# LouisBearing/BirdSoundClassif

Measured on AMD Instinct MI355X. Metric: clips/sec (3 s @ 22.05 kHz) detect fwd, higher is better.
Workload: dtype f32; 1 GPU; BASELINE.json configs[1]: 1xMI355X inference, batch=64 synthetic 3 s clips (PCM16 @22.05 kHz resident in HBM) through the HIP STFT front end + detector forward + device post-processing, detections returned to the host; batch_per_gpu=64, distinct_clips=64, lanes=2

## Files before the change

birdsoundclassif_amd/_lib.py:

```python
import ctypes as C
import os
import subprocess

_HERE = os.path.dirname(os.path.abspath(__file__))
LIB_PATH = os.environ.get('NBM_LIB') or os.path.join(_HERE, 'libnbm_hip.so')
CSRC = os.path.join(_HERE, 'csrc')

_lib = None


class GemmDesc(C.Structure):
    _fields_ = [('x', C.c_void_p), ('w', C.c_void_p), ('y', C.c_void_p),
                ('scale', C.c_void_p), ('shift', C.c_void_p), ('residual', C.c_void_p),
                ('x_gs', C.c_int64), ('w_gs', C.c_int64), ('y_gs', C.c_int64), ('res_gs', C.c_int64),
                ('groups', C.c_int),
                ('B', C.c_int), ('H', C.c_int), ('W', C.c_int), ('Cin', C.c_int),
                ('N', C.c_int),
                ('kh', C.c_int), ('kw', C.c_int), ('stride', C.c_int), ('pad', C.c_int),
                ('Ho', C.c_int), ('Wo', C.c_int),
                ('x_ld', C.c_int), ('w_ld', C.c_int), ('y_ld', C.c_int), ('res_ld', C.c_int),
                ('alpha', C.c_float), ('act', C.c_int), ('shift_per_row', C.c_int),
                ('up', C.c_void_p), ('up_H', C.c_int), ('up_W', C.c_int),
                ('rows', C.c_void_p), ('rows_blocks', C.c_void_p),
                ('rows_mode', C.c_int), ('rows_count', C.c_int), ('rows_TH', C.c_int), ('rows_TW', C.c_int),
# ... 76 lines not shown
    'nbm_upsample_bilinear_add': [_P, _I, _I, _I, _I, _P, _P, _I, _I, _P],
    'nbm_softmax_rows': [_P, _L, _I, _L, _P],
    'nbm_dwconv3x3': [_P, _I, _I, _I, _I, _I, _I, _P, _P, _P, _L, _P, _I, _I, _P],
    'nbm_silu': [_P, _P, _L, _P],
    'nbm_layernorm': [_P, _L, _I, _P, _P, _F, _P, _P],
    'nbm_mha_small': [_P, _P, _P, _I, _I, _I, _P, _I, _I, _I, _I, _I, _L, _L, _P, _F, _P],
    'nbm_mha_segments': [_P, _P, _P, _I, _I, _I, _P, _I, _I, _I, _I, _I, _I, _P, _P, _I, _F, _P],
    'nbm_pair_softmax': [_P, _L, _I, _I, _P, _I, _P],
    'nbm_rpn_decode': [_P, _P, _P, _I, _I, _I, _I, _I, _I, _P, _P, _P, _P],
    'nbm_nan_images': [_P, _I, _L, _P, _P],
    'nbm_rpn_select': [_P, _P, _P, _I, _I, _I, _I, _I, _P, _P, _P, _P, _P],
    'nbm_nms_batched': [_P, _P, _P, _I, _I, _F, _I, _P, _P, _P, _P, _P, _P, _P],
    'nbm_rpn_select_big_workspace': [_I, _I, C.POINTER(C.c_int64)],
    'nbm_rpn_select_big': [_P, _P, _P, _I, _I, _I, _I, _I, _P, _L, _P, _P, _P, _P, _P],
    'nbm_nms_big_workspace': [_I, _I, C.POINTER(C.c_int64)],
    'nbm_nms_big': [_P, _P, _P, _I, _I, _F, _I, _P, _L, _P, _P, _P, _P, _P],
    'nbm_roi_pool': [C.POINTER(RoiDesc), _P],
    'nbm_rcnn_post': [_P, _P, _I, _I, _P, _P, _I, _I, _I, _F, _F, _I, _P, _P, _P],
    'nbm_merge_collect': [_P, _P, _I, _I, _I, _I, _I, _L, _P, _P, _P, _P, _P, _P],
    'nbm_merge_nms_workspace': [_I, C.POINTER(C.c_int64)],
    'nbm_merge_nms': [_P, _P, _I, _F, _P, _L, _P, _P, _P],
    'nbm_merge_gather': [_P, _P, _P, _P, _P, _I, _P, _P, _P],
    'nbm_conv_dgrad': [C.POINTER(BwdDesc), _P],
    'nbm_conv_wgrad': [C.POINTER(BwdDesc), _P],
    'nbm_gemm_plan': [_I, _P, C.POINTER(GemmPlan)],
    'nbm_relu_bwd': [_P, _P, _P, _L, _P],
    'nbm_silu_bwd': [_P, _P, _P, _L, _P],
    'nbm_axpby': [_P, _P, _P, _F, _F, _L, _L, _P],
    'nbm_colsum': [_P, _L, _I, _I, _P, _P],
    'nbm_leaky_relu_bwd': [_P, _P, _P, _F, _L, _P],
    'nbm_layernorm_bwd': [_P, _P, _P, _L, _I, _F, _P, _P, _P, _P],
    'nbm_mha_small_bwd': [_P, _P, _P, _P, _I, _I, _I, _I, _P, _P, _P, _I, _I, _I, _P, _I, _I, _I, _I, _L, _L, _P, _F, _P],
    'nbm_zero_roi_windows': [_P, _I, _I, _I, _P, _P, _I, _I, _I, _P],
    'nbm_zero_pattern': [_P, _I, _I, _I, _I, _I, _P],
    'nbm_zero_tiles': [_P, _I, _I, _I, _I, _P, _I, _P, _P],
    'nbm_tiles_gather': [_P, _I, _I, _I, _I, _P, _I, _P, _P, _P],
    'nbm_tiles_scatter_add': [_P, _I, _I, _I, _I, _P, _I, _P, _P, _P],
    'nbm_proposal_iou': [_P, _P, _P, _I, _I, _I, _P, _P, _P],
    'nbm_anchor_targets': [_P, _I, _P, _P, _I, _I, _F, _F, _P, _P, _P, _P],
    'nbm_maxpool3x3s2_bwd': [_P, _P, _P, _I, _I, _I, _I, _I, _I, _P, _P, _P],
    'nbm_upsample_bilinear_bwd': [_P, _I, _I, _I, _I, _P, _I, _I, _I, _P],
    'nbm_tiles_upsample_bilinear_bwd_add': [_P, _I, _I, _I, _I, _P, _I, _P, _P, _I, _I, _P],
    'nbm_png_unfilter_gray8': [_P, _L, _I, _I, _I, _P, _L, _P, _P],
    'nbm_image_half_std_u8': [_P, _L, _I, _L, _P, _P],
    'nbm_randn_fill': [_U64, _L, _P, _P],
    'nbm_augment_batch': [_P, _P, _P, _I, _I, _I, _P, _P, _P, _P, _P, _P, _P],
    'nbm_u8_to_unit': [_P, _L, _P, _P],
    'nbm_wino_input': [_P, _I, _I, _I, _I, _P, _I, _P],
    'nbm_wino_output': [_P, _P, _P, _P, _I, _I, _I, _I, _I, _P, _I, _P, _P],
    'nbm_wino_outgrad': [_P, _I, _I, _I, _I, _P, _P, _I, _P],
    'nbm_wino_weight': [_P, _P, _I, _I, _I, _I, _P, _P],
    'nbm_wino_weight_grad': [_P, _P, _I, _I, _I, _P, _P],
    'nbm_wino23_rows': [_P, _I, _I, _I, _I, _P, _P],
    'nbm_wino23_conv_fused': [_P, _P, _P, _P, _P, _I, _I, _I, _I, _I, _I, _P, _I, _P],
    'nbm_wino23_rows_tiles': [_P, _I, _I, _I, _I, _P, _I, _P, _P, _P, _I, _P],
    'nbm_wino23_conv_fused_tiles': [_P, _P, _P, _P, _P, _I, _I, _I, _I, _I, _I, _P, _P, _I, _P, _P, _P],
    'nbm_roi_tiles': [_P, _P, _I, _I, _I, _I, _P, _P, _P, _I, _P, _P, _P],
    'nbm_wino23_input_tiles': [_P, _I, _I, _I, _I, _P, _I, _P, _P, _P],
    'nbm_wino23_outgrad_tiles': [_P, _I, _I, _I, _I, _P, _I, _P, _P, _P, _I, _P],
    'nbm_cell_outgrad': [_P, _I, _I, _I, _I, _I, _P, _P, _P],
    'nbm_cell_weight': [_P, _I, _I, _P, _I, _P, _I, _P],
    'nbm_cell_weight_fold': [_P, _P, _I, _I, _I, _I, _F, _P, _I, _P, _I, _P],
    'nbm_cell_weight_grad': [_P, _I, _I, _I, _P, _P],
    'nbm_cell_input': [_P, _I, _I, _I, _I, _I, _P, _I, _I, _P],
    'nbm_cell_input_up': [_P, _P, _I, _I, _I, _I, _I, _I, _I, _P, _I, _I, _P],
    'nbm_cell_patches': [_P, _I, _I, _I, _I, _I, _P, _I, _I, _P],
    'nbm_cell_patches_up': [_P, _P, _I, _I, _I, _I, _I, _I, _I, _P, _I, _I, _P],
    'nbm_cell_patches_up_cols': [_P, _P, _I, _I, _I, _I, _I, _I, _I, _P, _P],
    'nbm_cell_dgrad_output': [_P, _I, _I, _I, _I, _I, _P, _I, _I, _I, _P, _P],
    'nbm_cell_output': [_P, _P, _I, _I, _I, _I, _I, _P, _P],
    'nbm_weighted_sum': [_P, _P, _P, _P, _P, _L, _P],
    'nbm_weighted_sum_bwd': [_P, _P, _P, _P, _P, _P, _P, _P, _P, _L, _P],
    'nbm_softmax_rows_bwd': [_P, _P, _P, _L, _I, _F, _P],
    'nbm_pair_softmax_bwd': [_P, _P, _P, _L, _P],
    'nbm_dwconv3x3_bwd': [_P, _P, _P, _I, _I, _I, _I, _I, _I, _P, _P, _P, _I, _I, _P],
    'nbm_dwconv3x3_bwd_acc': [_P, _P, _I, _I, _I, _I, _I, _I, _P, _I, _I, _P],
    'nbm_film_fwd': [_P, _P, _P, _L, _I, _P],
    'nbm_film_bwd': [_P, _P, _P, _P, _P, _L, _I, _P],
    'nbm_bn_train_fwd': [_P, _L, _I, _P, _P, _F, _F, _P, _P, _P, _P, _P, _P, _P],
    'nbm_bn_train_bwd': [_P, _P, _L, _I, _P, _P, _P, _P, _P, _P, _P, _P],
    'nbm_roi_pool_bwd': [C.POINTER(C.c_void_p), C.POINTER(C.c_int), C.POINTER(C.c_int), _I, _I, _P, _P, _I, _I, _P, _P],
    'nbm_sqnorm_accum': [_P, _L, _P, _P],
    'nbm_adamw_step': [_P, _P, _P, _P, _L, _F, _F, _F, _F, _F, _I, _P, _F, _P],
}


def build(verbose=False):
    r = subprocess.run(['make', '-C', CSRC, '-j4'], capture_output=True, text=True)
    if verbose or r.returncode:
        print(r.stdout[-4000:], r.stderr[-4000:])
    if r.returncode:
        raise RuntimeError('building libnbm_hip.so failed')
    return LIB_PATH


def load():
    global _lib
    if _lib is not None:
        return _lib
    import torch
    if not os.path.isfile(LIB_PATH):
        raise RuntimeError(f'{LIB_PATH} is missing: build it with `python -c "import __graft_entry__ as g; g.build()"` '
                           '(the NBM hot path has no CPU / eager fallback)')
    lib = C.CDLL(LIB_PATH)
    lib.nbm_version.restype = C.c_char_p
    lib.nbm_version.argtypes = []
# ... 20 lines not shown
```

birdsoundclassif_amd/csrc/wino_fused.hip:

```cpp
#include "nbm_common.h"
#include "igemm_device.h"
#include <type_traits>

namespace {

constexpr int BK = 32;
constexpr int PITCH = 36;
constexpr int LIST_BM = 128;

struct WinoFusedParams {
  const float* R; const float* U; float* y;
  const float* scale; const float* shift; const float* mask;
  long long r_gs;
  int u_gs;
  int T, N, C, nk;
  int H, W, TH, TW, THW, WP;
  nbm_fastdiv fd_thw, fd_tw;
  int m_tiles, n_tiles, relu;
  const int* tiles; const int* n_blocks;
  const unsigned* blk_info;
};

__global__ __launch_bounds__(256) void wino23_rows_kernel(const float* __restrict__ x, int B, int H, int W, int C4,
                                                          int TH, int WP, float* __restrict__ R) {
  const long long per_plane = (long long)B * TH * WP * C4;
  const f32x4* x4 = reinterpret_cast<const f32x4*>(x);
  f32x4* r4 = reinterpret_cast<f32x4*>(R);
  const f32x4 zero = {0.f, 0.f, 0.f, 0.f};
  for (long long idx = blockIdx.x * 256ll + threadIdx.x; idx < per_plane; idx += (long long)gridDim.x * 256) {
    const int c = (int)(idx % C4);
    long long t = idx / C4;
    const int xp = (int)(t % WP);
    t /= WP;
    const int ty = (int)(t % TH), b = (int)(t / TH);
    const int ix = xp - 1;
    f32x4 d[4];
#pragma unroll
    for (int a = 0; a < 4; ++a) {
      const int iy = 2 * ty - 1 + a;
      const bool ok = (unsigned)iy < (unsigned)H && (unsigned)ix < (unsigned)W;
      d[a] = ok ? x4[(((long long)b * H + iy) * W + ix) * C4 + c] : zero;
    }
    r4[idx] = d[0] - d[2];
    r4[idx + per_plane] = d[1] + d[2];
    r4[idx + 2 * per_plane] = d[2] - d[1];
    r4[idx + 3 * per_plane] = d[1] - d[3];
  }
}

__global__ __launch_bounds__(256) void wino23_rows_tiles_kernel(const float* __restrict__ x, int B, int H, int W, int C4,
                                                                int TH, int TW, int WP, const int* __restrict__ tiles,
                                                                int n_entries, const int* __restrict__ n_blocks,
                                                                const unsigned* __restrict__ blk_info, float* __restrict__ R,
                                                                int pat_stride) {
  const int S = pat_stride, OHp = S > 0 ? (H + 2 - 3) / S + 1 : 0, OWp = S > 0 ? (W + 2 - 3) / S + 1 : 0;
  const long long per_plane = (long long)B * TH * WP * C4;
  const f32x4* x4 = reinterpret_cast<const f32x4*>(x);
  f32x4* r4 = reinterpret_cast<f32x4*>(R);
  const f32x4 zero = {0.f, 0.f, 0.f, 0.f};
  if (n_blocks) n_entries = min(n_entries, *n_blocks * LIST_BM);
  const long long total = (long long)n_entries * 4 * C4;
  for (long long idx = blockIdx.x * 256ll + threadIdx.x; idx < total; idx += (long long)gridDim.x * 256) {
    const int c = (int)(idx % C4);
    const long long t = idx / C4;
    const int k = (int)(t & 3), e = (int)(t >> 2);
    const int id = tiles[e];
    if (id < 0) continue;
    const unsigned pm = blk_info ? blk_info[e >> 7] & 0xffffu : 0xffffu;
    if ((k == 0 && !(pm & 0x1111u)) || (k == 3 && !(pm & 0x8888u))) continue;
    const int THW = TH * TW;
    const int b = id / THW, rem = id - b * THW;
    const int ty = rem / TW, tx = rem - ty * TW;
    const int xp = 2 * tx + k, ix = xp - 1;
    f32x4 d[4];
#pragma unroll
    for (int a = 0; a < 4; ++a) {
      const int iy = 2 * ty - 1 + a;
      bool ok = (unsigned)iy < (unsigned)H && (unsigned)ix < (unsigned)W &&
                !(a == 0 && !(pm & 0x000fu)) && !(a == 3 && !(pm & 0xf000u));
      if (S > 0 && ok && (iy + 1) % S < 3 && (iy + 1) / S < OHp && (ix + 1) % S < 3 && (ix + 1) / S < OWp) ok = false;
      d[a] = ok ? x4[(((long long)b * H + iy) * W + ix) * C4 + c] : zero;
    }
    const long long o = (((long long)b * TH + ty) * WP + xp) * C4 + c;
    if (pm & 0x000fu) r4[o] = d[0] - d[2];
    r4[o + per_plane] = d[1] + d[2];
    r4[o + 2 * per_plane] = d[2] - d[1];
    if (pm & 0xf000u) r4[o + 3 * per_plane] = d[1] - d[3];
  }
}

template <int BM, int BN, int WM, int WN>
__global__ __launch_bounds__(256, BN == 128 ? 1 : 2) void wino23_fused_kernel(const WinoFusedParams p) {
  constexpr int MT = WM / 32, NT = WN / 32;
  constexpr int WAVES_N = BN / WN;
  constexpr int AR = BM / 32, BR = BN / 32;
  static_assert((BM / WM) * WAVES_N == 4, "4 waves per workgroup");

  __shared__ __attribute__((aligned(16))) float lds[2 * (BM + BN) * PITCH];
  if constexpr (BN != 128) nbm_stagger_priority();
  float* As = lds;
  float* Bs = lds + 2 * BM * PITCH;

  const int wg = xcd_tile(gridDim.x, blockIdx.x);
  int tile_m = wg / p.n_tiles, tile_n = wg - tile_m * p.n_tiles;
  if (p.n_blocks) {
    const int j = blockIdx.x >> 3;
    tile_n = j % p.n_tiles;
    tile_m = (j / p.n_tiles) * 8 + (blockIdx.x & 7);
    if (tile_m >= p.m_tiles) return;
  }
  const int bm0 = tile_m * BM, bn0 = tile_n * BN;

  if (p.tiles) {
    if (p.n_blocks && tile_m >= *p.n_blocks) return;
    if (p.tiles[bm0] < 0) return;
  }
  auto tile_of = [&](int t) { return p.tiles ? p.tiles[t] : t; };
  const unsigned info = (p.tiles && p.blk_info) ? p.blk_info[tile_m] : 0x000fffffu;
  const unsigned plane_mask = info & 0xffffu, store_mask = (info >> 16) & 0xfu;

  const int tid = threadIdx.x, lane = tid & 63, wave = tid >> 6;
  const int wm0 = (wave / WAVES_N) * WM, wn0 = (wave % WAVES_N) * WN;
  const int lrow = lane & 31, lh = lane >> 5;
  const int c4 = tid & 7, r0 = tid >> 3;

  unsigned a_rel[AR], b_rel[BR];
  long long blk_base;
  {
    const int t = bm0 < p.T ? tile_of(bm0) : 0;
    const int bi = (int)nbm_fdiv((unsigned)t, p.fd_thw), rem = t - bi * p.THW;
    const int ty = (int)nbm_fdiv((unsigned)rem, p.fd_tw), tx = rem - ty * p.TW;
    blk_base = (((long long)bi * p.TH + ty) * p.WP + 2 * tx) * p.C;
  }
#pragma unroll
  for (int i = 0; i < AR; ++i) {
    const int t = bm0 + r0 + 32 * i < p.T ? tile_of(bm0 + r0 + 32 * i) : -1;
    if (t >= 0) {
      const int bi = (int)nbm_fdiv((unsigned)t, p.fd_thw), rem = t - bi * p.THW;
      const int ty = (int)nbm_fdiv((unsigned)rem, p.fd_tw), tx = rem - ty * p.TW;
      const long long off = (((long long)bi * p.TH + ty) * p.WP + 2 * tx) * p.C - blk_base;
      a_rel[i] = (unsigned)((off + c4 * 4) * 4);
    } else {
      a_rel[i] = 0x80000000u;
    }
  }
#pragma unroll
  for (int i = 0; i < BR; ++i) {
    const int n = bn0 + r0 + 32 * i;
    b_rel[i] = n < p.N ? (unsigned)((n * p.C + c4 * 4) * 4) : 0x80000000u;
  }
  const float* a_plane0 = p.R + blk_base;
  const __amdgpu_buffer_rsrc_t rsrc_b = make_rsrc(p.U, 0x7ffffff0u);

  f32x4 ra[AR], ra2[AR], rb[BR];
  float a_sign = 1.f;
  unsigned ld_rem = plane_mask;
  int ld_xi = __builtin_ctz(ld_rem), ld_c0 = 0;

  auto load_tiles = [&]() {
    const int i = ld_xi >> 2, j = ld_xi & 3;
    const int k1 = j == 0 ? 0 : (j == 2 ? 2 : 1), k2 = j == 2 ? 1 : (j == 3 ? 3 : 2);
    const __amdgpu_buffer_rsrc_t rsrc_a = make_rsrc(a_plane0 + (long long)i * p.r_gs, 0x7ffffff0u);
    const unsigned a_soff1 = (unsigned)((k1 * p.C + ld_c0) * 4), a_soff2 = (unsigned)((k2 * p.C + ld_c0) * 4);
    const unsigned b_soff = (unsigned)((ld_xi * p.u_gs + ld_c0) * 4);
#pragma unroll
    for (int r = 0; r < AR; ++r) {
      ra[r] = __builtin_bit_cast(f32x4, __builtin_amdgcn_raw_buffer_load_b128(rsrc_a, a_rel[r], a_soff1, 0));
      ra2[r] = __builtin_bit_cast(f32x4, __builtin_amdgcn_raw_buffer_load_b128(rsrc_a, a_rel[r], a_soff2, 0));
    }
#pragma unroll
    for (int r = 0; r < BR; ++r)
      rb[r] = __builtin_bit_cast(f32x4, __builtin_amdgcn_raw_buffer_load_b128(rsrc_b, b_rel[r], b_soff, 0));
    ld_c0 += BK;
    if (ld_c0 == p.C) { ld_c0 = 0; ld_rem &= ld_rem - 1; ld_xi = ld_rem ? __builtin_ctz(ld_rem) : 0; }
  };
  unsigned st_rem = plane_mask;
  int st_xi = __builtin_ctz(st_rem), st_c0 = 0;
  auto store_lds = [&](int buf) {
    const float sgn = (st_xi & 3) == 1 ? 1.f : -1.f;
#pragma unroll
    for (int r = 0; r < AR; ++r) {
      f32x4 v;
#pragma unroll
      for (int e = 0; e < 4; ++e) v[e] = fmaf(sgn, ra2[r][e], ra[r][e]);
      *reinterpret_cast<f32x4*>(As + (buf * BM + r0 + 32 * r) * PITCH + c4 * 4) = v;
    }
#pragma unroll
    for (int r = 0; r < BR; ++r)
      *reinterpret_cast<f32x4*>(Bs + (buf * BN + r0 + 32 * r) * PITCH + c4 * 4) = rb[r];
    st_c0 += BK;
    if (st_c0 == p.C) { st_c0 = 0; st_rem &= st_rem - 1; st_xi = st_rem ? __builtin_ctz(st_rem) : 0; }
  };
  (void)a_sign;

  f32x16 acc[MT][NT];
  f32x16 Y[2][2][MT][NT];
#pragma unroll
  for (int i = 0; i < MT; ++i)
#pragma unroll
    for (int j = 0; j < NT; ++j)
#pragma unroll
      for (int e = 0; e < 16; ++e) {
        acc[i][j][e] = 0.f;
        Y[0][0][i][j][e] = 0.f; Y[0][1][i][j][e] = 0.f; Y[1][0][i][j][e] = 0.f; Y[1][1][i][j][e] = 0.f;
      }

  f32x4 fa[2][MT], fb[2][NT];
  auto read_frags = [&](const float* Ab, const float* Bb, int q, int s) {
#pragma unroll
    for (int i = 0; i < MT; ++i) fa[s][i] = *reinterpret_cast<const f32x4*>(Ab + i * 32 * PITCH + q * 4);
#pragma unroll
    for (int j = 0; j < NT; ++j) fb[s][j] = *reinterpret_cast<const f32x4*>(Bb + j * 32 * PITCH + q * 4);
  };
  auto mfma_group = [&](int s) {
#pragma unroll
    for (int e = 0; e < 4; ++e)
#pragma unroll
      for (int i = 0; i < MT; ++i)
#pragma unroll
        for (int j = 0; j < NT; ++j)
          acc[i][j] = __builtin_amdgcn_mfma_f32_32x32x2f32(fa[s][i][e], fb[s][j][e], acc[i][j], 0, 0, 0);
  };

  int cur = 0;
  auto k_step = [&](auto store_c, auto load_c) {
    constexpr bool STORE = decltype(store_c)::value, LOAD = decltype(load_c)::value;
    constexpr int NM = 4 * MT * NT;
    __syncthreads();
    const float* Ab = As + (cur * BM + wm0 + lrow) * PITCH + lh * 16;
    const float* Bb = Bs + (cur * BN + wn0 + lrow) * PITCH + lh * 16;
    read_frags(Ab, Bb, 0, 0);
    read_frags(Ab, Bb, 1, 1);
    mfma_group(0);
    if constexpr (STORE) store_lds(cur ^ 1);
    __builtin_amdgcn_sched_group_barrier(0x100, 2 * (MT + NT), 0);
    if constexpr (STORE) {
#pragma unroll
      for (int z = 0; z < AR + BR; ++z) {
        __builtin_amdgcn_sched_group_barrier(0x008, NM / (AR + BR) > 0 ? NM / (AR + BR) : 1, 0);
        __builtin_amdgcn_sched_group_barrier(0x200, 1, 0);
      }
    }
    __builtin_amdgcn_sched_barrier(0);
    read_frags(Ab, Bb, 2, 0);
    mfma_group(1);
    if constexpr (LOAD) load_tiles();
    __builtin_amdgcn_sched_group_barrier(0x100, MT + NT, 0);
    if constexpr (LOAD) {
#pragma unroll
      for (int z = 0; z < 2 * AR + BR; ++z) {
        __builtin_amdgcn_sched_group_barrier(0x008, 1, 0);
        __builtin_amdgcn_sched_group_barrier(0x002, 2, 0);
        __builtin_amdgcn_sched_group_barrier(0x020, 1, 0);
      }
    }
    __builtin_amdgcn_sched_barrier(0);
    read_frags(Ab, Bb, 3, 1);
    mfma_group(0);
    __builtin_amdgcn_sched_group_barrier(0x100, MT + NT, 0);
    __builtin_amdgcn_sched_group_barrier(0x008, NM, 0);
    __builtin_amdgcn_sched_barrier(0);
    mfma_group(1);
    cur ^= 1;
  };

  auto flush = [&](int xi) {
    const int i = xi >> 2, j = xi & 3;
    const float ai[2] = {i < 3 ? 1.f : 0.f, i == 0 ? 0.f : (i == 1 ? 1.f : -1.f)};
    const float aj[2] = {j < 3 ? 1.f : 0.f, j == 0 ? 0.f : (j == 1 ? 1.f : -1.f)};
#pragma unroll
    for (int pp = 0; pp < 2; ++pp)
#pragma unroll
      for (int qq = 0; qq < 2; ++qq) {
        const float c = ai[pp] * aj[qq];
        if (c != 0.f) {
#pragma unroll
          for (int a = 0; a < MT; ++a)
#pragma unroll
            for (int b = 0; b < NT; ++b)
#pragma unroll
              for (int e = 0; e < 16; ++e) Y[pp][qq][a][b][e] = fmaf(c, acc[a][b][e], Y[pp][qq][a][b][e]);
        }
      }
#pragma unroll
    for (int a = 0; a < MT; ++a)
#pragma unroll
      for (int b = 0; b < NT; ++b)
#pragma unroll
        for (int e = 0; e < 16; ++e) acc[a][b][e] = 0.f;
  };

  using TT = std::true_type;
  using FF = std::false_type;
  load_tiles();
  store_lds(0);
  load_tiles();
  for (unsigned rem = plane_mask; rem;) {
    const int xi = __builtin_ctz(rem);
    rem &= rem - 1;
    if (rem) {
      for (int kt = 0; kt < p.nk; ++kt) k_step(TT{}, TT{});
    } else {
      for (int kt = 0; kt + 2 < p.nk; ++kt) k_step(TT{}, TT{});
      k_step(TT{}, FF{});
      k_step(FF{}, FF{});
    }
    flush(xi);
  }
  __syncthreads();

  constexpr int CP = BN + 4;
  static_assert(BM * CP + 2 * BM <= 2 * (BM + BN) * PITCH, "epilogue tile + row table must fit the operand buffers");
  float* Cs = lds;
  long long* row_pix = reinterpret_cast<long long*>(lds + BM * CP);
  if (tid < BM) {
    const int t = bm0 + tid < p.T ? tile_of(bm0 + tid) : -1;
    long long v = -1;
    if (t >= 0) {
      const int bi = (int)nbm_fdiv((unsigned)t, p.fd_thw), rem = t - bi * p.THW;
      const int ty = (int)nbm_fdiv((unsigned)rem, p.fd_tw), tx = rem - ty * p.TW;
      const long long pix = (p.relu & 4) ? (long long)(bm0 + tid) * 4 : ((long long)bi * p.H + 2 * ty) * p.W + 2 * tx;
      v = (pix << 2) | (2 * ty + 1 < p.H ? 2 : 0) | (2 * tx + 1 < p.W ? 1 : 0);
    }
    row_pix[tid] = v;
  }
  constexpr int CH = BN / 4;
  constexpr int RPP = 256 / CH;
  const int cc = tid % CH, rr = tid / CH;
  const int n = bn0 + cc * 4;
  f32x4 sc = {1.f, 1.f, 1.f, 1.f}, sh = {0.f, 0.f, 0.f, 0.f};
  if (n < p.N) {
    if (p.scale) sc = *reinterpret_cast<const f32x4*>(p.scale + n);
    if (p.shift) sh = *reinterpret_cast<const f32x4*>(p.shift + n);
  }
#pragma unroll
  for (int pp = 0; pp < 2; ++pp)
#pragma unroll
    for (int qq = 0; qq < 2; ++qq) {
      if (!((store_mask >> (2 * pp + qq)) & 1u)) continue;
      __syncthreads();
#pragma unroll
      for (int a = 0; a < MT; ++a)
#pragma unroll
        for (int b = 0; b < NT; ++b)
#pragma unroll
          for (int e = 0; e < 16; ++e)
            Cs[(wm0 + a * 32 + (e & 3) + 8 * (e >> 2) + 4 * lh) * CP + wn0 + b * 32 + lrow] = Y[pp][qq][a][b][e];
      __syncthreads();
      if (n < p.N) {
        const int need = (pp ? 2 : 0) | (qq ? 1 : 0);
#pragma unroll 4
        for (int r = rr; r < BM; r += RPP) {
          const long long rp = row_pix[r];
// ... 4 lines not shown
#pragma unroll
          for (int e = 0; e < 4; ++e) v[e] = v[e] * sc[e] + sh[e];
          if (p.relu & 1) {
#pragma unroll
            for (int e = 0; e < 4; ++e) v[e] = fmaxf(v[e], 0.f);
          }
          if (p.relu & 2) {
            const f32x4 o = *reinterpret_cast<const f32x4*>(p.y + idx);
            v[0] += o[0]; v[1] += o[1]; v[2] += o[2]; v[3] += o[3];
          }
          if (p.mask) {
            const f32x4 mk = *reinterpret_cast<const f32x4*>(p.mask + idx);
#pragma unroll
            for (int e = 0; e < 4; ++e) if (!(mk[e] > 0.f)) v[e] = 0.f;
          }
          *reinterpret_cast<f32x4*>(p.y + idx) = v;
        }
      }
    }
}

}

extern "C" int nbm_wino23_rows(const float* x, int B, int H, int W, int C, float* R, void* stream) {
  if (!x || !R || B <= 0 || H <= 0 || W <= 0 || C <= 0 || (C & 3)) return NBM_EINVAL;
  if (!nbm_aligned16(x) || !nbm_aligned16(R)) return NBM_EALIGN;
  const int TH = (H + 1) >> 1, TW = (W + 1) >> 1, WP = 2 * TW + 2;
  const long long n = (long long)B * TH * WP * (C / 4);
  long long g = (n + 255) / 256;
  if (g > 65536) g = 65536;
  hipLaunchKernelGGL(wino23_rows_kernel, dim3((unsigned)g), dim3(256), 0, (hipStream_t)stream, x, B, H, W, C / 4, TH, WP, R);
  return nbm_launch_status();
}

extern "C" int nbm_wino23_rows_tiles(const float* x, int B, int H, int W, int C, const int* tiles, int n_entries,
                                     const int* n_blocks, const unsigned* blk_info, float* R, int skip_pattern_stride,
                                     void* stream) {
  if (!x || !R || !tiles || B <= 0 || H <= 0 || W <= 0 || C <= 0 || (C & 3) || n_entries < 0 || skip_pattern_stride < 0) return NBM_EINVAL;
  if (!nbm_aligned16(x) || !nbm_aligned16(R)) return NBM_EALIGN;
  if (n_entries == 0) return NBM_OK;
  const int TH = (H + 1) >> 1, TW = (W + 1) >> 1, WP = 2 * TW + 2;
  const long long n = (long long)n_entries * 4 * (C / 4);
  long long g = (n + 255) / 256;
  if (g > 16384) g = 16384;
  hipLaunchKernelGGL(wino23_rows_tiles_kernel, dim3((unsigned)g), dim3(256), 0, (hipStream_t)stream, x, B, H, W, C / 4, TH, TW,
                     WP, tiles, n_entries, n_blocks, blk_info, R, skip_pattern_stride);
  return nbm_launch_status();
}

static int wino23_conv_fused_launch(const float* R, const float* U, const float* scale, const float* shift,
                                    const float* mask, int relu, int B, int H, int W, int C, int N, float* y,
                                    const int* tiles, int n_entries, const int* n_blocks, const unsigned* blk_info,
                                    int variant, void* stream);

extern "C" int nbm_wino23_conv_fused(const float* R, const float* U, const float* scale, const float* shift,
                                     const float* mask, int relu, int B, int H, int W, int C, int N, float* y,
                                     int variant, void* stream) {
  return wino23_conv_fused_launch(R, U, scale, shift, mask, relu, B, H, W, C, N, y, nullptr, 0, nullptr, nullptr, variant, stream);
}

extern "C" int nbm_wino23_conv_fused_tiles(const float* R, const float* U, const float* scale, const float* shift,
                                           const float* mask, int relu, int B, int H, int W, int C, int N, float* y,
                                           const int* tiles, int n_entries, const int* n_blocks, const unsigned* blk_info,
                                           void* stream) {
  if (!tiles || n_entries < 0 || (n_entries % LIST_BM)) return NBM_EINVAL;
  if (n_entries == 0) return NBM_OK;
  return wino23_conv_fused_launch(R, U, scale, shift, mask, relu, B, H, W, C, N, y, tiles, n_entries, n_blocks, blk_info, 0,
                                  stream);
}

static int wino23_conv_fused_launch(const float* R, const float* U, const float* scale, const float* shift,
                                    const float* mask, int relu, int B, int H, int W, int C, int N, float* y,
                                    const int* tiles, int n_entries, const int* n_blocks, const unsigned* blk_info,
                                    int variant, void* stream) {
  if (!R || !U || !y || B <= 0 || H <= 0 || W <= 0 || C <= 0 || N <= 0) return NBM_EINVAL;
  if ((C % BK) || C / BK < 2 || (N & 3)) return NBM_EUNSUPPORTED;
  if (!nbm_aligned16(R) || !nbm_aligned16(U) || !nbm_aligned16(y) || (shift && !nbm_aligned16(shift)) ||
      (scale && !nbm_aligned16(scale)) || (mask && !nbm_aligned16(mask)))
    return NBM_EALIGN;
  WinoFusedParams p{};
  p.TH = (H + 1) >> 1; p.TW = (W + 1) >> 1; p.THW = p.TH * p.TW; p.WP = 2 * p.TW + 2;
  p.fd_thw = nbm_fastdiv_make((unsigned)p.THW); p.fd_tw = nbm_fastdiv_make((unsigned)p.TW);
  const long long T = (long long)B * p.THW;
  if (T > 0x7fffff00ll || (long long)N * C * 16 * 4 > 0x7fffffffll) return NBM_EUNSUPPORTED;
  if ((130ll * p.WP + 4) * C * 4 > 0x7fffffffll) return NBM_EUNSUPPORTED;
  if (tiles && (long long)(B < 8 ? B : 8) * p.TH * p.WP * C * 4 > 0x7fffffffll) return NBM_EUNSUPPORTED;
  p.R = R; p.U = U; p.y = y; p.scale = scale; p.shift = shift; p.mask = mask; p.relu = relu;
  p.T = (int)T; p.N = N; p.C = C; p.nk = C / BK; p.H = H; p.W = W;
  p.r_gs = (long long)B * p.TH * p.WP * C; p.u_gs = N * C;
  p.m_tiles = (int)((T + LIST_BM - 1) / LIST_BM);
  p.tiles = tiles; p.n_blocks = n_blocks; p.blk_info = blk_info;
  if (tiles) { p.T = n_entries; p.m_tiles = n_entries / LIST_BM; }
  hipStream_t st = (hipStream_t)stream;
  if (variant != 0 && variant != 64 && variant != 128) return NBM_EINVAL;
  const bool wide = variant == 128 || (variant == 0 && N % 128 == 0);
  p.n_tiles = wide ? (N + 127) / 128 : (N + 63) / 64;
  int bm = LIST_BM;
  if (wide && !tiles) {
    const char* fe = getenv("NBM_WINO_BM");
    const int force = fe ? atoi(fe) : 0;
    static const int cus = [] { int dev = 0, n = 0; (void)hipGetDevice(&dev); (void)hipDeviceGetAttribute(&n, hipDeviceAttributeMultiprocessorCount, dev);
                                return n > 0 ? n : 256; }();
    const long long nt = p.n_tiles;
    const long long r128 = ((T + 127) / 128 * nt + cus - 1) / cus, r96 = ((T + 95) / 96 * nt + cus - 1) / cus;
    if (force == 96 || (force == 0 && r96 * 96 * 108 < r128 * 128 * 100)) bm = 96;
    if (force == 128) bm = 128;
    p.m_tiles = (int)((T + bm - 1) / bm);
  }
  const dim3 grid((n_blocks ? (p.m_tiles + 7) / 8 * 8 : p.m_tiles) * p.n_tiles), block(256);
#define NBM_WF(BM_, BN_, WM_, WN_) hipLaunchKernelGGL((wino23_fused_kernel<BM_, BN_, WM_, WN_>), grid, block, 0, st, p)
  if (!wide) NBM_WF(128, 64, 64, 32);
  else if (bm == 96) NBM_WF(96, 128, 96, 32);
  else NBM_WF(128, 128, 64, 64);
#undef NBM_WF
  return nbm_launch_status();
}
```

birdsoundclassif_amd/ops.py:

```python
import collections
import ctypes as C
import os
import math

import torch

from . import _lib
from ._lib import GconvBwdDesc, GconvDesc, GemmDesc, RoiDesc, check

ACT_NONE, ACT_RELU, ACT_SILU, ACT_LEAKY = 0, 1, 2, 3

PROFILE = None
FLOPS = None
FLOPS_DEFERRED = []


def flops_total():
    tot = FLOPS[0] + sum(float(c.item()) * f for c, f in FLOPS_DEFERRED)
    FLOPS_DEFERRED.clear()
    return tot


_PROFILE_LABEL = None
PROFILE_ONLY = None
# ... 892 lines not shown

def unpack_merged(out):
    out = out.cpu() if out.is_cuda else out
    n = int(out[:1].view(torch.int32)[0])
    return out[1:1 + 6 * n].view(n, 6)


from ._lib import BwdDesc


class _timed:

    def __init__(self, tag):
        self.tag = tag

    def __enter__(self):
        if PROFILE_BWD is not None:
            self.ev = (torch.cuda.Event(enable_timing=True), torch.cuda.Event(enable_timing=True))
            self.ev[0].record()

    def __exit__(self, *exc):
        if PROFILE_BWD is not None:
            self.ev[1].record()
            PROFILE_BWD.append((self.tag, *self.ev))


PROFILE_BWD = None


def _bwd_desc(g, *, B, H, W, Cin, N, kh, kw, stride, pad, g_ld, groups=1, alpha=1.0):
    d = BwdDesc()
    d.g = g.data_ptr()
    d.groups = groups
    d.B, d.H, d.W, d.Cin, d.N = B, H, W, Cin, N
    d.kh, d.kw, d.stride, d.pad = kh, kw, stride, pad
    d.Ho = (H + 2 * pad - kh) // stride + 1
    d.Wo = (W + 2 * pad - kw) // stride + 1
    d.g_ld = g_ld
    d.alpha = float(alpha)
    return d


GemmPlan = collections.namedtuple('GemmPlan', 'rc kernel grid block m_tiles n_tiles vec_epi fast slices phased ph_tiles splits k_chunk '
                                              'plain b_generic narrow_m halves')


def gemm_plan(kind, desc):
    p = _lib.GemmPlan()
    lib().nbm_gemm_plan(int(kind), C.byref(desc), C.byref(p))
    return GemmPlan(p.rc, (p.name or b'').decode(), tuple(p.grid), p.block, p.m_tiles, p.n_tiles, p.vec_epi, p.fast, p.slices, p.phased,
                    tuple(p.ph_tiles), p.splits, p.k_chunk, p.plain, p.b_generic, p.narrow_m, p.halves)


def split_nn():
    return os.environ.get('NBM_SPLIT_BF16') == '1' and os.environ.get('NBM_SPLIT_NN', '1') != '0'


def conv_dgrad(g, w, out, *, B, H, W, Cin, N, kh=1, kw=1, stride=1, pad=0, g_ld=None, w_ld=None, out_ld=None,
               a_scale=None, residual=None, mask=None, alpha=1.0, groups=1, g_gs=0, w_gs=0, out_gs=0, res_gs=0, residual2=None,
               mask_bits=None):
    if (kh == 1 and kw == 1 and stride == 1 and pad == 0 and residual2 is None and N > 256 and N % 32 == 0 and Cin > 64 and Cin % 4 == 0 and
            (groups == 1 or (mask is None and a_scale is None)) and split_nn()):
        wl = kh * kw * Cin if w_ld is None else w_ld
        wv = w.as_strided((groups, N, Cin), (w_gs, wl, 1))
        wt = (wv * a_scale[None, :N, None] if a_scale is not None else wv).transpose(1, 2).contiguous()
        with _timed(('dgrad', B, H, W, Cin, N, kh, stride, groups)):
            gemm_conv(g, wt, out, B=B, H=H, W=W, Cin=N, N=Cin, x_ld=N if g_ld is None else g_ld, w_ld=N,
                      y_ld=Cin if out_ld is None else out_ld, residual=residual, res_ld=Cin if residual is not None else None, alpha=alpha,
                      mask=mask, mask_ld=Cin if mask is not None else None, groups=groups, x_gs=g_gs, w_gs=Cin * N, y_gs=out_gs, res_gs=res_gs)
        return out
    d = _bwd_desc(g, B=B, H=H, W=W, Cin=Cin, N=N, kh=kh, kw=kw, stride=stride, pad=pad,
                  g_ld=N if g_ld is None else g_ld, groups=groups, alpha=alpha)
    d.w, d.out = w.data_ptr(), out.data_ptr()
    d.w_ld = kh * kw * Cin if w_ld is None else w_ld
    d.out_ld = Cin if out_ld is None else out_ld
    d.a_scale = a_scale.data_ptr() if a_scale is not None else None
    d.residual = residual.data_ptr() if residual is not None else None
    d.res_ld = Cin if residual is not None else 0
    d.mask = mask.data_ptr() if mask is not None else None
    d.mask_ld = Cin if mask is not None else 0
    if mask_bits is not None and groups == 1 and Cin % 32 == 0:
        assert mask_bits.dtype == torch.int32 and mask_bits.numel() * 32 >= B * H * W * Cin
        d.mask_bits, d.mask, d.mask_ld = mask_bits.data_ptr(), None, 0
    if residual2 is not None:
        if groups != 1 or tuple(residual2.shape) != (B, (H + 1) // 2, (W + 1) // 2, Cin) or kh != 1 or stride != 1:
            raise ValueError('conv_dgrad: residual2 must be [B, ceil(H/2), ceil(W/2), Cin] of a 1x1 / stride-1 data gradient')
        d.residual2, d.res2_ld = _chk(residual2, name='residual2').data_ptr(), Cin
    d.g_gs, d.w_gs, d.out_gs, d.res_gs = g_gs, w_gs, out_gs, res_gs
    if FLOPS is not None:
        FLOPS[0] += 2.0 * B * d.Ho * d.Wo * N * kh * kw * Cin * groups
    with _timed(('dgrad', B, H, W, Cin, N, kh, stride, groups)):
        check(lib().nbm_conv_dgrad(C.byref(d), _stream()), 'nbm_conv_dgrad')
    return out


def conv_wgrad(g, x, out, *, B, H, W, Cin, N, kh=1, kw=1, stride=1, pad=0, g_ld=None, x_ld=None, out_ld=None,
               row_scale=None, alpha=1.0, groups=1, g_gs=0, x_gs=0, out_gs=0, bias_grad=None):
    d = _bwd_desc(g, B=B, H=H, W=W, Cin=Cin, N=N, kh=kh, kw=kw, stride=stride, pad=pad,
                  g_ld=N if g_ld is None else g_ld, groups=groups, alpha=alpha)
    d.x, d.out = x.data_ptr(), out.data_ptr()
    d.x_ld = Cin if x_ld is None else x_ld
    d.out_ld = kh * kw * Cin if out_ld is None else out_ld
    d.row_scale = row_scale.data_ptr() if row_scale is not None else None
    d.g_gs, d.x_gs, d.out_gs = g_gs, x_gs, out_gs
    deferred_bias = None
    if bias_grad is not None and groups == 1:
# ... 364 lines not shown
```

include/nbm_hip.h:

```cpp
#ifndef NBM_HIP_H
#define NBM_HIP_H

#include <stdint.h>

#ifdef __cplusplus
extern "C" {
#endif

#define NBM_OK 0
#define NBM_EINVAL (-1)
#define NBM_EALIGN (-2)
#define NBM_EUNSUPPORTED (-3)

#define NBM_ACT_NONE 0
#define NBM_ACT_RELU 1
#define NBM_ACT_SILU 2
#define NBM_ACT_LEAKY 3

const char* nbm_version(void);

int nbm_graph_census(void* graph, long long counts[6]);

typedef struct nbm_gemm_desc {
  const float* x;
// ... 19 lines not shown
  int rows_mode, rows_count, rows_TH, rows_TW;
  const float* mask;
  int mask_ld;
  unsigned* bits_out;
} nbm_gemm_desc;

int nbm_gemm_conv(const nbm_gemm_desc* d, void* stream);

typedef struct nbm_gconv_desc {
  const float* x;
  const float* w;
  float* y;
  const float* scale;
  const float* shift;
  int B, H, W;
  int groups, Cg;
  int kh, kw, stride, pad;
  int Ho, Wo;
  int x_ld, y_ld;
  int relu;
} nbm_gconv_desc;
int nbm_gconv3x3(const nbm_gconv_desc* d, void* stream);

typedef struct nbm_gconv_bwd_desc {
  const float* g;
  const float* y;
  const float* w;
  const float* x;
  float* out;
  const float* scale;
  void* workspace;
  long long workspace_bytes;
  int B, H, W;
  int groups, Cg;
  int kh, kw, stride, pad;
  int Ho, Wo;
  int g_ld, y_ld, x_ld, out_ld;
  int accumulate;
  int splits;
} nbm_gconv_bwd_desc;
int nbm_gconv3x3_dgrad(const nbm_gconv_bwd_desc* d, void* stream);
int nbm_gconv3x3_wgrad(const nbm_gconv_bwd_desc* d, void* stream);
int nbm_gconv3x3_wgrad_workspace(const nbm_gconv_bwd_desc* d, long long* bytes);

int nbm_wino_input(const float* x, int B, int H, int W, int C, float* V, int m, void* stream);
int nbm_wino_output(const float* M, const float* scale, const float* shift, const float* mask, int relu, int B, int H, int W,
                    int N, float* y, int m, const float* residual, void* stream);
int nbm_wino_outgrad(const float* g, int B, int H, int W, int N, float* dM, float* bias_grad, int m, void* stream);

int nbm_wino_weight(const float* g, const float* scale, int N, int C, int transposed, int m, float* U, void* stream);
int nbm_wino_weight_grad(const float* dU, const float* row_scale, int N, int C, int m, float* dW, void* stream);

int nbm_wino23_rows(const float* x, int B, int H, int W, int C, float* R, void* stream);
int nbm_wino23_conv_fused(const float* R, const float* U, const float* scale, const float* shift, const float* mask,
                          int relu, int B, int H, int W, int C, int N, float* y, int variant, void* stream);

int nbm_wino23_rows_tiles(const float* x, int B, int H, int W, int C, const int* tiles, int n_entries, const int* n_blocks,
                          const unsigned* blk_info, float* R,
                          int skip_pattern_stride ,
                          void* stream);
int nbm_wino23_conv_fused_tiles(const float* R, const float* U, const float* scale, const float* shift, const float* mask,
                                int relu ,
                                int B, int H, int W, int C, int N, float* y, const int* tiles, int n_entries,
                                const int* n_blocks, const unsigned* blk_info, void* stream);
int nbm_roi_tiles(const float* rois, const int* n_roi, int B, int roi_cap, int n_levels, int level, const int* fh,
                  const int* fw, const unsigned char* skip, int dilate, int* tiles, int* n_blocks, void* stream);
int nbm_wino23_input_tiles(const float* x, int B, int H, int W, int C, const int* tiles, int n_list, const unsigned* plane_mask,
                           float* V, void* stream);
int nbm_wino23_outgrad_tiles(const float* g, int B, int H, int W, int N, const int* tiles, int n_list, const unsigned* plane_mask,
                             float* dM, float* bias_grad, int skip_pattern_stride, void* stream);
int nbm_cell_outgrad(const float* g, int B, int H, int W, int N, int stride, float* Vg, float* bias_grad, void* stream);
int nbm_cell_weight(const float* w, int N, int C, float* U_nc, int ld, float* U_cn, int ldt, void* stream);
int nbm_cell_weight_fold(const float* w, const float* w_lat, int wl_ld, int N, int C, int Cin, float alpha, float* U_nc, int ld,
                         float* U_cn, int ldt, void* stream);
int nbm_cell_weight_grad(const float* dU, int N, int C, int ld, float* dW, void* stream);
int nbm_cell_input(const float* x, int B, int H, int W, int C, int stride, float* Vx, int ld ,
                   int c_off , void* stream);
int nbm_cell_input_up(const float* x1, const float* bias, int B, int H, int W, int C, int Hc, int Wc, int stride, float* Vx, int ld,
                      int c_off, void* stream);
int nbm_cell_patches(const float* x, int B, int H, int W, int C, int stride, float* Vx, int ld, int c_off, void* stream);
int nbm_cell_patches_up(const float* x1, const float* bias, int B, int H, int W, int C, int Hc, int Wc, int stride, float* Vx, int ld,
                        int c_off, void* stream);
int nbm_cell_patches_up_cols(const float* x1, const float* bias, int B, int H, int W, int C, int Hc, int Wc, int stride, float* Vx,
                             void* stream);

int nbm_copy_rect(float* strided, float* packed, int64_t n_outer, int64_t outer_pitch, int n_rows, int64_t row_pitch, int64_t width,
                  int to_strided, int zero_strided, void* stream);
int nbm_cell_dgrad_output(const float* M, int B, int H, int W, int C, int stride, float* gx, int parity_class,
                          int ld , int c_off ,
                          float* bias_grad , void* stream);
int nbm_cell_output(const float* M, const float* bias, int B, int H, int W, int N, int stride, float* y, void* stream);


int nbm_pcm16_to_wave(const int16_t* pcm, int64_t pcm_ld, int batch, int n, int upsample,
                      const int32_t* hq, int64_t first, int64_t count, float* out, int64_t out_ld, int lead,
                      int pad_mode, void* stream);

int nbm_resample_to_wave(const float* x, int64_t x_ld, int batch, int64_t n, int L, int M, const double* taps, int T,
                         int64_t first, int64_t count, float* out, int64_t out_ld, int lead, int pad_mode, int quant16,
                         void* stream);

#define NBM_WAV_MAX_CHANNELS 8
int nbm_wav_decode(const void* raw, int64_t raw_pitch, int batch, int tag, int bits, int channels, int64_t n, float* out,
                   int64_t out_pitch, void* stream);

int nbm_minmax_init(uint32_t* minmax, int batch, void* stream);
// ... 231 lines not shown
```

Baseline: 1060 clips/s.

## Add 64-row Winograd fused tile variant with two workgroups per CU

Adds a BM=64, BN=128 variant of the fused Winograd F(2,3) GEMM kernel that allows two workgroups per CU. Listed (tile-driven) launches are split so each 128-entry list block becomes two halves, and the LDS staging layout and pipeline tail are reorganised for this variant. Tile-shape selection moves into a shared cost model that also weighs the 64-row option for dense launches. The aim is better occupancy and wave balance on the sparse ROI and dense convolutions, at the cost of less reuse per workgroup and more blocks to launch.

```diff
diff --git a/birdsoundclassif_amd/_lib.py b/birdsoundclassif_amd/_lib.py
--- a/birdsoundclassif_amd/_lib.py
+++ b/birdsoundclassif_amd/_lib.py
@@ -152,6 +152,7 @@
     'nbm_wino_weight': [_P, _P, _I, _I, _I, _I, _P, _P],
     'nbm_wino_weight_grad': [_P, _P, _I, _I, _I, _P, _P],
     'nbm_wino23_rows': [_P, _I, _I, _I, _I, _P, _P],
+    'nbm_wino23_fused_shape': [_L, _I, _I, _I, C.POINTER(C.c_int), C.POINTER(C.c_int), C.POINTER(C.c_int)],
     'nbm_wino23_conv_fused': [_P, _P, _P, _P, _P, _I, _I, _I, _I, _I, _I, _P, _I, _P],
     'nbm_wino23_rows_tiles': [_P, _I, _I, _I, _I, _P, _I, _P, _P, _P, _I, _P],
     'nbm_wino23_conv_fused_tiles': [_P, _P, _P, _P, _P, _I, _I, _I, _I, _I, _I, _P, _P, _I, _P, _P, _P],
diff --git a/birdsoundclassif_amd/csrc/wino_fused.hip b/birdsoundclassif_amd/csrc/wino_fused.hip
--- a/birdsoundclassif_amd/csrc/wino_fused.hip
+++ b/birdsoundclassif_amd/csrc/wino_fused.hip
@@ -1,5 +1,6 @@
 #include "nbm_common.h"
 #include "igemm_device.h"
+#include "wino_plan.h"
 #include <type_traits>
 
 namespace {
@@ -90,14 +91,15 @@
 }
 
 template <int BM, int BN, int WM, int WN>
-__global__ __launch_bounds__(256, BN == 128 ? 1 : 2) void wino23_fused_kernel(const WinoFusedParams p) {
+__global__ __launch_bounds__(256, (BN == 128 && BM > 64) ? 1 : 2) void wino23_fused_kernel(const WinoFusedParams p) {
   constexpr int MT = WM / 32, NT = WN / 32;
+  constexpr int HALVES = BM == 64 ? LIST_BM / BM : 1;
   constexpr int WAVES_N = BN / WN;
   constexpr int AR = BM / 32, BR = BN / 32;
   static_assert((BM / WM) * WAVES_N == 4, "4 waves per workgroup");
 
   __shared__ __attribute__((aligned(16))) float lds[2 * (BM + BN) * PITCH];
-  if constexpr (BN != 128) nbm_stagger_priority();
+  if constexpr (BN != 128 || BM == 64) nbm_stagger_priority();
   float* As = lds;
   float* Bs = lds + 2 * BM * PITCH;
 
@@ -106,17 +108,19 @@
   if (p.n_blocks) {
     const int j = blockIdx.x >> 3;
     tile_n = j % p.n_tiles;
-    tile_m = (j / p.n_tiles) * 8 + (blockIdx.x & 7);
+    const int jm = j / p.n_tiles;
+    tile_m = ((jm / HALVES) * 8 + (blockIdx.x & 7)) * HALVES + jm % HALVES;
     if (tile_m >= p.m_tiles) return;
   }
   const int bm0 = tile_m * BM, bn0 = tile_n * BN;
+  const int blk = tile_m / HALVES;
 
   if (p.tiles) {
-    if (p.n_blocks && tile_m >= *p.n_blocks) return;
+    if (p.n_blocks && blk >= *p.n_blocks) return;
     if (p.tiles[bm0] < 0) return;
   }
   auto tile_of = [&](int t) { return p.tiles ? p.tiles[t] : t; };
-  const unsigned info = (p.tiles && p.blk_info) ? p.blk_info[tile_m] : 0x000fffffu;
+  const unsigned info = (p.tiles && p.blk_info) ? p.blk_info[blk] : 0x000fffffu;
   const unsigned plane_mask = info & 0xffffu, store_mask = (info >> 16) & 0xfu;
 
   const int tid = threadIdx.x, lane = tid & 63, wave = tid >> 6;
@@ -176,18 +180,27 @@
   };
   unsigned st_rem = plane_mask;
   int st_xi = __builtin_ctz(st_rem), st_c0 = 0;
-  auto store_lds = [&](int buf) {
+  constexpr bool LEAN = BM == 64;
+  auto st_at = [&](float* base, int rows, int stage, int r) {
+    if constexpr (LEAN) return base + (stage * (rows / BM) + (r0 * PITCH + c4 * 4) + r * (32 * PITCH));
+    else return base + (stage * rows + r0 + 32 * r) * PITCH + c4 * 4;
+  };
+  auto rd_at = [&](const float* base, int rows, int stage, int w0) {
+    if constexpr (LEAN) return base + (stage * (rows / BM) + w0 * PITCH + (lrow * PITCH + lh * 16));
+    else return base + (stage * rows + w0 + lrow) * PITCH + lh * 16;
+  };
+  auto store_lds = [&](int stage) {
     const float sgn = (st_xi & 3) == 1 ? 1.f : -1.f;
 #pragma unroll
     for (int r = 0; r < AR; ++r) {
       f32x4 v;
 #pragma unroll
       for (int e = 0; e < 4; ++e) v[e] = fmaf(sgn, ra2[r][e], ra[r][e]);
-      *reinterpret_cast<f32x4*>(As + (buf * BM + r0 + 32 * r) * PITCH + c4 * 4) = v;
+      *reinterpret_cast<f32x4*>(st_at(As, BM, stage, r)) = v;
     }
 #pragma unroll
     for (int r = 0; r < BR; ++r)
-      *reinterpret_cast<f32x4*>(Bs + (buf * BN + r0 + 32 * r) * PITCH + c4 * 4) = rb[r];
+      *reinterpret_cast<f32x4*>(st_at(Bs, BN, stage, r)) = rb[r];
     st_c0 += BK;
     if (st_c0 == p.C) { st_c0 = 0; st_rem &= st_rem - 1; st_xi = st_rem ? __builtin_ctz(st_rem) : 0; }
   };
@@ -223,16 +236,17 @@
   };
 
   int cur = 0;
+  constexpr int FLIP = LEAN ? BM * PITCH : 1;
   auto k_step = [&](auto store_c, auto load_c) {
     constexpr bool STORE = decltype(store_c)::value, LOAD = decltype(load_c)::value;
     constexpr int NM = 4 * MT * NT;
     __syncthreads();
-    const float* Ab = As + (cur * BM + wm0 + lrow) * PITCH + lh * 16;
-    const float* Bb = Bs + (cur * BN + wn0 + lrow) * PITCH + lh * 16;
+    const float* Ab = rd_at(As, BM, cur, wm0);
+    const float* Bb = rd_at(Bs, BN, cur, wn0);
     read_frags(Ab, Bb, 0, 0);
     read_frags(Ab, Bb, 1, 1);
     mfma_group(0);
-    if constexpr (STORE) store_lds(cur ^ 1);
+    if constexpr (STORE) store_lds(cur ^ FLIP);
     __builtin_amdgcn_sched_group_barrier(0x100, 2 * (MT + NT), 0);
     if constexpr (STORE) {
 #pragma unroll
@@ -261,7 +275,7 @@
     __builtin_amdgcn_sched_group_barrier(0x008, NM, 0);
     __builtin_amdgcn_sched_barrier(0);
     mfma_group(1);
-    cur ^= 1;
+    cur ^= FLIP;
   };
 
   auto flush = [&](int xi) {
@@ -298,7 +312,13 @@
   for (unsigned rem = plane_mask; rem;) {
     const int xi = __builtin_ctz(rem);
     rem &= rem - 1;
-    if (rem) {
+    if constexpr (LEAN) {
+      for (int kt = rem ? 0 : 2; kt < p.nk; ++kt) k_step(TT{}, TT{});
+      if (!rem) {
+        k_step(TT{}, FF{});
+        k_step(FF{}, FF{});
+      }
+    } else if (rem) {
       for (int kt = 0; kt < p.nk; ++kt) k_step(TT{}, TT{});
     } else {
       for (int kt = 0; kt + 2 < p.nk; ++kt) k_step(TT{}, TT{});
@@ -409,6 +429,14 @@
                                     const float* mask, int relu, int B, int H, int W, int C, int N, float* y,
                                     const int* tiles, int n_entries, const int* n_blocks, const unsigned* blk_info,
                                     int variant, void* stream);
+
+extern "C" int nbm_wino23_fused_shape(long long T, int N, int cus, int listed, int* bm, int* bn, int* wg_per_cu) {
+  if (T <= 0 || N <= 0 || cus <= 0 || !bm || !bn || !wg_per_cu) return NBM_EINVAL;
+  const char* fe = getenv("NBM_WINO_BM");
+  const nbm_wino::FusedShape sh = nbm_wino::fused_shape(T, N, cus, listed != 0, 0, fe ? atoi(fe) : 0);
+  *bm = sh.bm; *bn = sh.bn; *wg_per_cu = sh.wg_per_cu;
+  return NBM_OK;
+}
 
 extern "C" int nbm_wino23_conv_fused(const float* R, const float* U, const float* scale, const float* shift,
                                      const float* mask, int relu, int B, int H, int W, int C, int N, float* y,
@@ -450,24 +478,18 @@
   if (tiles) { p.T = n_entries; p.m_tiles = n_entries / LIST_BM; }
   hipStream_t st = (hipStream_t)stream;
   if (variant != 0 && variant != 64 && variant != 128) return NBM_EINVAL;
-  const bool wide = variant == 128 || (variant == 0 && N % 128 == 0);
-  p.n_tiles = wide ? (N + 127) / 128 : (N + 63) / 64;
-  int bm = LIST_BM;
-  if (wide && !tiles) {
-    const char* fe = getenv("NBM_WINO_BM");
-    const int force = fe ? atoi(fe) : 0;
-    static const int cus = [] { int dev = 0, n = 0; (void)hipGetDevice(&dev); (void)hipDeviceGetAttribute(&n, hipDeviceAttributeMultiprocessorCount, dev);
-                                return n > 0 ? n : 256; }();
-    const long long nt = p.n_tiles;
-    const long long r128 = ((T + 127) / 128 * nt + cus - 1) / cus, r96 = ((T + 95) / 96 * nt + cus - 1) / cus;
-    if (force == 96 || (force == 0 && r96 * 96 * 108 < r128 * 128 * 100)) bm = 96;
-    if (force == 128) bm = 128;
-    p.m_tiles = (int)((T + bm - 1) / bm);
-  }
-  const dim3 grid((n_blocks ? (p.m_tiles + 7) / 8 * 8 : p.m_tiles) * p.n_tiles), block(256);
+  const char* fe = getenv("NBM_WINO_BM");
+  static const int cus = [] { int dev = 0, n = 0; (void)hipGetDevice(&dev); (void)hipDeviceGetAttribute(&n, hipDeviceAttributeMultiprocessorCount, dev);
+                              return n > 0 ? n : 256; }();
+  const nbm_wino::FusedShape sh = nbm_wino::fused_shape(p.T, N, cus, tiles != nullptr, variant, fe ? atoi(fe) : 0);
+  p.n_tiles = (N + sh.bn - 1) / sh.bn;
+  p.m_tiles = tiles ? n_entries / LIST_BM * (LIST_BM / sh.bm) : (int)((T + sh.bm - 1) / sh.bm);
+  const int per_blk = tiles ? LIST_BM / sh.bm : 1;
+  const dim3 grid((n_blocks ? (p.m_tiles / per_blk + 7) / 8 * 8 * per_blk : p.m_tiles) * p.n_tiles), block(256);
 #define NBM_WF(BM_, BN_, WM_, WN_) hipLaunchKernelGGL((wino23_fused_kernel<BM_, BN_, WM_, WN_>), grid, block, 0, st, p)
-  if (!wide) NBM_WF(128, 64, 64, 32);
-  else if (bm == 96) NBM_WF(96, 128, 96, 32);
+  if (sh.bn == 64) NBM_WF(128, 64, 64, 32);
+  else if (sh.bm == 96) NBM_WF(96, 128, 96, 32);
+  else if (sh.bm == 64) NBM_WF(64, 128, 32, 64);
   else NBM_WF(128, 128, 64, 64);
 #undef NBM_WF
   return nbm_launch_status();
diff --git a/birdsoundclassif_amd/csrc/wino_plan.h b/birdsoundclassif_amd/csrc/wino_plan.h
--- /dev/null
+++ b/birdsoundclassif_amd/csrc/wino_plan.h
@@ -0,0 +1,28 @@
+#pragma once
+
+namespace nbm_wino {
+
+struct FusedShape { int bm, bn, wg_per_cu; };
+
+constexpr int PEN_128 = 100, PEN_96 = 108, PEN_64 = 97, PEN_64_ALONE = 108;
+
+inline long long cu_blocks(long long T, int nt, int cus, int bm) { return ((T + bm - 1) / bm * nt + cus - 1) / cus; }
+
+inline FusedShape fused_shape(long long T, int N, int cus, bool listed, int variant = 0, int force_bm = 0) {
+  const bool wide = variant == 128 || (variant == 0 && N % 128 == 0);
+  if (!wide) return {128, 64, 2};
+  const FusedShape s128{128, 128, 1}, s96{96, 128, 1}, s64{64, 128, 2};
+  if (listed) return force_bm == 128 ? s128 : s64;
+  if (force_bm == 128) return s128;
+  if (force_bm == 96) return s96;
+  if (force_bm == 64) return s64;
+  if (cus <= 0) cus = 256;
+  const int nt = (N + 127) / 128;
+  const long long n64 = cu_blocks(T, nt, cus, 64);
+  const long long c128 = cu_blocks(T, nt, cus, 128) * 128 * PEN_128, c96 = cu_blocks(T, nt, cus, 96) * 96 * PEN_96,
+                  c64 = n64 * 64 * (n64 >= 2 ? PEN_64 : PEN_64_ALONE);
+  if (c64 < c128 && c64 < c96) return s64;
+  return c96 < c128 ? s96 : s128;
+}
+
+}
diff --git a/birdsoundclassif_amd/ops.py b/birdsoundclassif_amd/ops.py
--- a/birdsoundclassif_amd/ops.py
+++ b/birdsoundclassif_amd/ops.py
@@ -968,6 +968,13 @@
                     tuple(p.ph_tiles), p.splits, p.k_chunk, p.plain, p.b_generic, p.narrow_m, p.halves)
 
 
+def wino23_fused_shape(T, N, cus=256, listed=False):
+    bm, bn, wpc = C.c_int(), C.c_int(), C.c_int()
+    check(lib().nbm_wino23_fused_shape(int(T), int(N), int(cus), int(bool(listed)), C.byref(bm), C.byref(bn), C.byref(wpc)),
+          'nbm_wino23_fused_shape')
+    return bm.value, bn.value, wpc.value
+
+
 def split_nn():
     return os.environ.get('NBM_SPLIT_BF16') == '1' and os.environ.get('NBM_SPLIT_NN', '1') != '0'
 
diff --git a/include/nbm_hip.h b/include/nbm_hip.h
--- a/include/nbm_hip.h
+++ b/include/nbm_hip.h
@@ -95,6 +95,7 @@
 int nbm_wino_weight_grad(const float* dU, const float* row_scale, int N, int C, int m, float* dW, void* stream);
 
 int nbm_wino23_rows(const float* x, int B, int H, int W, int C, float* R, void* stream);
+int nbm_wino23_fused_shape(long long T, int N, int cus, int listed, int* bm, int* bn, int* wg_per_cu);
 int nbm_wino23_conv_fused(const float* R, const float* U, const float* scale, const float* shift, const float* mask,
                           int relu, int B, int H, int W, int C, int N, float* y, int variant, void* stream);
 
```

Result: no change. 1062 clips/s (median of 5 runs) (+0.2%).
